# ChainSafe/co-zkvms

Hardware: AMD Instinct MI355X
Metric: RISC-V cycles proved/sec (co-Jolt hot path: PST13 commit + dense GKR grand product + openings) (higher is better)
Workload: dtype u32-limb BN254 Fr/Fq (254-bit Montgomery integers); 1 GPU; configs[1] restated (SURVEY 8d): 2^20-cycle trace per GPU, plain prover, 128 polys (64 Fr + 32 u16 + 16 u32 + 16 flags) PST13 batch commit, dense grand product 8 x 2^21 leaves, batch evaluate + opening reduction + PST13 open; log_n=20, polys=128, gp_batch=8, parallelism=single GPU, ranks_per_gpu=1

## Files before the change

### co-zkvms_amd/csrc/common.hpp

```cpp
#pragma once
#ifdef COZK_COUNT_COPIES
#include <hip/hip_runtime.h>
#include <map>
#include <string>
#include <cstdio>
#include <mutex>
struct CozkCopyCounter {
    std::map<std::string, unsigned long> m;
    std::mutex mu;
    ~CozkCopyCounter() {
        for (auto& kv : m) fprintf(stderr, "[copies] %8lu  %s\n", kv.second, kv.first.c_str());
    }
};
inline CozkCopyCounter& cozk_copy_counter() { static CozkCopyCounter c; return c; }
inline void cozk_count_copy(const char* what, const char* f, int l) {
    auto& c = cozk_copy_counter();
    std::lock_guard<std::mutex> g(c.mu);
    const char* b = f;
    for (const char* p = f; *p; p++) if (*p == '/') b = p + 1;
    c.m[std::string(what) + " " + b + ":" + std::to_string(l)]++;
}
#define hipMemcpyAsync(...) (cozk_count_copy("memcpy", __FILE__, __LINE__), hipMemcpyAsync(__VA_ARGS__))
#define hipStreamSynchronize(...) (cozk_count_copy("sync", __FILE__, __LINE__), hipStreamSynchronize(__VA_ARGS__))
#define hipMemsetAsync(...) (cozk_count_copy("memset", __FILE__, __LINE__), hipMemsetAsync(__VA_ARGS__))
// ... 186 lines not shown
    ProfSlot prof_slots[COZK_PROF_SLOTS];
    void* ring_comm = nullptr;
    int ring_rank = 0, ring_n = 0;
    uint64_t ring_bytes = 0;
};

struct ProfScope {
    cozk_ctx* ctx;
    hipStream_t st;
    int slot;
    hipEvent_t e0 = nullptr, e1 = nullptr;
    ProfScope(cozk_ctx* c, int slot_, uint64_t alg_bytes, hipStream_t stream = nullptr) : ctx(c), st(stream ? stream : c->stream), slot(slot_) {
        if (!ctx->prof_enabled) return;
        if (hipEventCreate(&e0) != hipSuccess || hipEventCreate(&e1) != hipSuccess) {
            e0 = e1 = nullptr;
            return;
        }
        (void)hipEventRecord(e0, st);
        ctx->prof_slots[slot].launches += 1;
        ctx->prof_slots[slot].alg_bytes += alg_bytes;
    }
    ~ProfScope() {
        if (!e0) return;
        (void)hipEventRecord(e1, st);
        ctx->prof_slots[slot].events.push_back({e0, e1});
    }
};

struct cozk_bases {
    cozk_ctx* ctx;
    size_t n;
    int nwin;
    g1_affine* table;
    bool has_inf = true;
};

struct cozk_vec {
    cozk_ctx* ctx;
    size_t n;
    int kind;
    void* d;
    size_t bytes;
    bool owned;
};

static inline size_t scalar_kind_bytes(int kind) {
    switch (kind) {
        case COZK_SCALAR_FR: return 32;
        case COZK_SCALAR_U8: return 1;
        case COZK_SCALAR_U16: return 2;
        case COZK_SCALAR_U32: return 4;
        case COZK_SCALAR_U64: return 8;
        case COZK_SCALAR_I64: return 8;
        default: return 0;
    }
}

inline std::mutex g_ctx_mu;
inline std::unordered_set<cozk_ctx*> g_live_ctx;
inline thread_local cozk_ctx* t_cur_ctx = nullptr;
static inline void trim_current_pool() {
    if (t_cur_ctx) t_cur_ctx->pool.trim();
}
static inline bool ctx_is_live(cozk_ctx* ctx) {
    std::lock_guard<std::mutex> lk(g_ctx_mu);
    return g_live_ctx.count(ctx) != 0;
// ... 56 lines not shown
```

### co-zkvms_amd/csrc/msm.hip

```cpp
#include "common.hpp"
#include "fq9.hip.hpp"

static constexpr uint32_t NB = 1u << 15;
static constexpr int CH = 16;
static constexpr int TPB = 256;

template <int KIND>
struct ScalarKind;
template <>
struct ScalarKind<COZK_SCALAR_FR> {
    static constexpr int NWIN = 16;
    static __device__ __forceinline__ bool load(const void* p, size_t i, uint32_t w[8]) {
        fe s = Fr::from_mont(fe_load(reinterpret_cast<const fe*>(p) + i));
#pragma unroll
        for (int k = 0; k < 8; k++) w[k] = s.l[k];
        return false;
    }
};
template <>
struct ScalarKind<COZK_SCALAR_U8> {
    static constexpr int NWIN = 1;
    static __device__ __forceinline__ bool load(const void* p, size_t i, uint32_t w[8]) {
        w[0] = reinterpret_cast<const uint8_t*>(p)[i];
        return false;
// ... 21 lines not shown
    static constexpr int NWIN = 5;
    static __device__ __forceinline__ bool load(const void* p, size_t i, uint32_t w[8]) {
        uint64_t v = reinterpret_cast<const uint64_t*>(p)[i];
        w[0] = (uint32_t)v;
        w[1] = (uint32_t)(v >> 32);
        w[2] = 0;
        return false;
    }
};
template <>
struct ScalarKind<COZK_SCALAR_I64> {
    static constexpr int NWIN = 5;
    static __device__ __forceinline__ bool load(const void* p, size_t i, uint32_t w[8]) {
        int64_t v = reinterpret_cast<const int64_t*>(p)[i];
        bool neg = v < 0;
        uint64_t m = neg ? (uint64_t)0 - (uint64_t)v : (uint64_t)v;
        w[0] = (uint32_t)m;
        w[1] = (uint32_t)(m >> 32);
        w[2] = 0;
        return neg;
    }
};

static inline int kind_nwin(int kind) {
    switch (kind) {
        case COZK_SCALAR_FR: return 16;
        case COZK_SCALAR_U8: return 1;
        case COZK_SCALAR_U16: return 2;
        case COZK_SCALAR_U32: return 3;
        default: return 5;
    }
}

template <int KIND, class F>
__device__ __forceinline__ void for_each_digit(const void* scalars, size_t i, F&& f) {
    uint32_t w[8] = {0, 0, 0, 0, 0, 0, 0, 0};
    bool neg = ScalarKind<KIND>::load(scalars, i, w);
    uint32_t carry = 0;
#pragma unroll
    for (int k = 0; k < ScalarKind<KIND>::NWIN; k++) {
        uint32_t v = ((w[k >> 1] >> (16 * (k & 1))) & 0xffffu) + carry;
        bool sub = v > 32768u;
        carry = sub ? 1u : 0u;
        uint32_t mag = sub ? 65536u - v : v;
        f(k, mag, sub != neg);
    }
}

static __device__ __forceinline__ uint32_t agg_atomic_add(uint32_t* counters, uint32_t key, bool active) {
    uint64_t act = __ballot(active);
    uint32_t pos = 0;
    if (act == 0) return 0;
    int lane = threadIdx.x & 63;
    int first = __ffsll((unsigned long long)act) - 1;
    uint32_t k0 = __shfl(key, first);
    uint64_t same = __ballot(active && key == k0);
    int cnt = __popcll(same);
    bool merged = false;
    if (cnt >= 4) {
        uint32_t base = 0;
        if (lane == first) base = atomicAdd(&counters[k0], (uint32_t)cnt);
        base = __shfl(base, first);
        if (active && key == k0) {
            pos = base + __popcll(same & ((1ull << lane) - 1ull));
            merged = true;
        }
    }
    if (active && !merged) pos = atomicAdd(&counters[key], 1u);
    return pos;
}
// ... 2 lines not shown
__global__ void __launch_bounds__(TPB) k_msm_hist(const void* scalars, size_t n, uint32_t* hist, int grouped) {
    size_t i = (size_t)blockIdx.x * TPB + threadIdx.x;
    bool inr = i < n;
    size_t ii = inr ? i : 0;
    for_each_digit<KIND>(scalars, ii, [&](int k, uint32_t mag, bool) {
        bool act = inr && mag != 0;
        uint32_t key = (grouped ? (uint32_t)k * NB : 0u) + (mag - 1u);
        agg_atomic_add(hist, act ? key : 0u, act);
    });
}

template <int KIND>
__global__ void __launch_bounds__(TPB) k_msm_scatter(const void* scalars, size_t n, uint32_t* cursor, uint32_t* refs,
                                                  int grouped, uint32_t table_n, uint32_t base_off) {
    size_t i = (size_t)blockIdx.x * TPB + threadIdx.x;
    bool inr = i < n;
    size_t ii = inr ? i : 0;
    for_each_digit<KIND>(scalars, ii, [&](int k, uint32_t mag, bool negative) {
        bool act = inr && mag != 0;
        uint32_t key = (grouped ? (uint32_t)k * NB : 0u) + (mag - 1u);
        uint32_t pos = agg_atomic_add(cursor, act ? key : 0u, act);
        if (act) {
            uint32_t ref = (grouped ? 0u : (uint32_t)k * table_n) + base_off + (uint32_t)ii;
            refs[pos] = ref | (negative ? 0x80000000u : 0u);
        }
    });
}

struct MsmPolyDesc {
    const void* scalars;
    uint32_t n;
    uint32_t base_off;
    uint32_t group;
    uint32_t pad;
};
static constexpr int LTPB = 1024;

template <int KIND>
__global__ void __launch_bounds__(LTPB) k_msm_hist_lds(const MsmPolyDesc* __restrict__ descs, uint32_t* __restrict__ hist) {
    __shared__ uint32_t lh[NB];
    const MsmPolyDesc d = descs[blockIdx.y];
    for (uint32_t b = threadIdx.x; b < NB; b += blockDim.x) lh[b] = 0;
    __syncthreads();
    for (size_t i = (size_t)blockIdx.x * blockDim.x + threadIdx.x; i < d.n; i += (size_t)gridDim.x * blockDim.x) {
        for_each_digit<KIND>(d.scalars, i, [&](int, uint32_t mag, bool) {
            if (mag != 0) atomicAdd(&lh[mag - 1u], 1u);
        });
    }
    __syncthreads();
    uint32_t* h = hist + (size_t)d.group * NB;
    for (uint32_t b = threadIdx.x; b < NB; b += blockDim.x) {
        uint32_t c = lh[b];
        if (c) atomicAdd(&h[b], c);
    }
}

template <int KIND>
__global__ void __launch_bounds__(LTPB) k_msm_scatter_lds(const MsmPolyDesc* __restrict__ descs, uint32_t* __restrict__ cursor,
                                                       uint32_t* __restrict__ refs, uint32_t table_n) {
    __shared__ uint32_t lh[NB];
    const MsmPolyDesc d = descs[blockIdx.y];
    for (uint32_t b = threadIdx.x; b < NB; b += blockDim.x) lh[b] = 0;
    __syncthreads();
    for (size_t i = (size_t)blockIdx.x * blockDim.x + threadIdx.x; i < d.n; i += (size_t)gridDim.x * blockDim.x) {
        for_each_digit<KIND>(d.scalars, i, [&](int, uint32_t mag, bool) {
            if (mag != 0) atomicAdd(&lh[mag - 1u], 1u);
        });
    }
    __syncthreads();
    uint32_t* cur = cursor + (size_t)d.group * NB;
    for (uint32_t b = threadIdx.x; b < NB; b += blockDim.x) {
        uint32_t c = lh[b];
        lh[b] = c ? atomicAdd(&cur[b], c) : 0u;
    }
    __syncthreads();
    for (size_t i = (size_t)blockIdx.x * blockDim.x + threadIdx.x; i < d.n; i += (size_t)gridDim.x * blockDim.x) {
        for_each_digit<KIND>(d.scalars, i, [&](int k, uint32_t mag, bool negative) {
            if (mag != 0) {
                uint32_t pos = atomicAdd(&lh[mag - 1u], 1u);
                uint32_t ref = (uint32_t)k * table_n + d.base_off + (uint32_t)i;
                refs[pos] = ref | (negative ? 0x80000000u : 0u);
            }
        });
    }
}

static constexpr uint32_t SCAN_PER_BLOCK = 1024;

template <bool FROM_OFFSETS>
static __device__ __forceinline__ void scan_load4(const uint32_t* __restrict__ in, uint32_t nb, uint32_t L, uint32_t b0, uint32_t c[4],
                                                  const uint32_t* __restrict__ perm) {
#pragma unroll
    for (int k = 0; k < 4; k++) {
        uint32_t b = b0 + k;
        if (b >= nb) c[k] = 0;
        else if (FROM_OFFSETS) {
            uint32_t q = perm ? perm[b] : b;
            c[k] = (in[q + 1] - in[q] + L - 1u) / L;
        } else c[k] = in[b];
    }
}

static __device__ __forceinline__ uint32_t block_exclusive_scan_256(uint32_t v, uint32_t* sh4, uint32_t* total) {
    uint32_t x = v;
#pragma unroll
    for (int off = 1; off < 64; off <<= 1) {
        uint32_t y = __shfl_up(x, off);
        if ((int)(threadIdx.x & 63) >= off) x += y;
    }
    int w = threadIdx.x >> 6;
    if ((threadIdx.x & 63) == 63) sh4[w] = x;
    __syncthreads();
    uint32_t base = 0;
    for (int i = 0; i < w; i++) base += sh4[i];
    if (total) *total = sh4[0] + sh4[1] + sh4[2] + sh4[3];
    __syncthreads();
    return base + x - v;
// ... 317 lines not shown
    g1_xyzz acc = G1::identity();
    for (uint32_t c = tid; c < cpg; c += TPB) acc = G1::add(acc, xyzz_load(chunk + (size_t)g * cpg + c));
    sh[tid] = acc;
    __syncthreads();
    for (uint32_t s = TPB / 2; s > 0; s >>= 1) {
        if (tid < s) {
            acc = G1::add(acc, sh[tid + s]);
            sh[tid] = acc;
        }
        __syncthreads();
    }
    if (tid == 0) xyzz_store(grp + g, acc);
}

__global__ void k_msm_finalize(const g1_xyzz* __restrict__ grp, uint32_t G, uint32_t npoly, g1_affine* __restrict__ out) {
    uint32_t p = blockIdx.x * blockDim.x + threadIdx.x;
    if (p >= npoly) return;
    g1_xyzz acc = xyzz_load(grp + (size_t)p * G + (G - 1));
    for (int w = (int)G - 2; w >= 0; w--) {
        for (int d = 0; d < 16; d++) acc = G1::dbl(acc);
        acc = G1::add(acc, xyzz_load(grp + (size_t)p * G + w));
    }
    affine_store(out + p, G1::to_affine(acc));
}

__global__ void __launch_bounds__(TPB) k_precompute_window(const g1_affine* __restrict__ prev, g1_affine* __restrict__ next, size_t n) {
    size_t i = (size_t)blockIdx.x * TPB + threadIdx.x;
    if (i >= n) return;
    g1_xyzz acc = G1::dbl_affine(affine_load(prev + i));
    for (int d = 1; d < 16; d++) acc = G1::dbl(acc);
    affine_store(next + i, G1::to_affine(acc));
}

__global__ void __launch_bounds__(TPB) k_fixed_base_mul(const fe* __restrict__ scalars, g1_affine g, g1_affine* __restrict__ out, size_t n) {
    size_t i = (size_t)blockIdx.x * TPB + threadIdx.x;
    if (i >= n) return;
    fe s = Fr::from_mont(fe_load(scalars + i));
    g1_xyzz acc = G1::identity();
    for (int k = 7; k >= 0; k--) {
        uint32_t w = s.l[k];
        for (int b = 31; b >= 0; b--) {
            acc = G1::dbl(acc);
            if ((w >> b) & 1u) acc = G1::add_mixed(acc, g);
        }
    }
    affine_store(out + i, G1::to_affine(acc));
}

__global__ void __launch_bounds__(TPB) k_pair_sums(const g1_affine* __restrict__ in, g1_affine* __restrict__ out, size_t nout) {
    size_t i = (size_t)blockIdx.x * TPB + threadIdx.x;
    if (i >= nout) return;
    g1_xyzz acc = G1::from_affine(affine_load(in + 2 * i));
    acc = G1::add_mixed(acc, affine_load(in + 2 * i + 1));
    affine_store(out + i, G1::to_affine(acc));
}

static inline uint32_t cdiv(uint64_t a, uint64_t b) { return (uint32_t)((a + b - 1) / b); }

__global__ void __launch_bounds__(TPB) k_any_infinity(const g1_affine* __restrict__ pts, size_t n, uint32_t* __restrict__ flag) {
    size_t i = (size_t)blockIdx.x * TPB + threadIdx.x;
    if (i < n && G1::is_inf(affine_load(pts + i))) atomicOr(flag, 1u);
}
static void build_window_table(cozk_ctx* ctx, cozk_bases* b) {
    for (int w = 1; w < b->nwin; w++) {
        k_precompute_window<<<cdiv(b->n, TPB), TPB, 0, ctx->stream>>>(b->table + (size_t)(w - 1) * b->n,
                                                                     b->table + (size_t)w * b->n, b->n);
    }
    HIP_TRY(hipGetLastError());
    ctx->scratch.reserve(64);
    uint32_t* flag = ctx->scratch.as<uint32_t>();
    HIP_TRY(hipMemsetAsync(flag, 0, 4, ctx->stream));
    k_any_infinity<<<cdiv(b->n, TPB), TPB, 0, ctx->stream>>>(b->table, b->n, flag);
    uint32_t h = 1;
    HIP_TRY(hipMemcpyAsync(&h, flag, 4, hipMemcpyDeviceToHost, ctx->stream));
    HIP_TRY(hipStreamSynchronize(ctx->stream));
    b->has_inf = h != 0;
}

#define KIND_DISPATCH(kind, CALL)                                              \
    switch (kind) {                                                            \
        case COZK_SCALAR_FR: { constexpr int K = COZK_SCALAR_FR; CALL; } break;   \
        case COZK_SCALAR_U8: { constexpr int K = COZK_SCALAR_U8; CALL; } break;   \
        case COZK_SCALAR_U16: { constexpr int K = COZK_SCALAR_U16; CALL; } break; \
        case COZK_SCALAR_U32: { constexpr int K = COZK_SCALAR_U32; CALL; } break; \
        case COZK_SCALAR_U64: { constexpr int K = COZK_SCALAR_U64; CALL; } break; \
        case COZK_SCALAR_I64: { constexpr int K = COZK_SCALAR_I64; CALL; } break; \
        default: throw CozkError(COZK_ERR_INVALID_ARG, "unknown scalar kind");    \
    }

struct MsmSetPlan {
    uint32_t P = 0, G = 1, nb = 0, L0 = 8;
    uint64_t M = 0, bound = 0, maxseg0 = 0;
    bool pre = false;
};

static MsmSetPlan msm_plan(const cozk_bases* bases, const size_t* offsets, const size_t* ns, const int* kinds, size_t P) {
    COZK_REQUIRE(P >= 1, "msm: empty batch");
    COZK_REQUIRE((uint64_t)bases->n * (uint64_t)bases->nwin < (1ull << 31), "msm: table too large for 31-bit refs");
    MsmSetPlan pl;
    pl.P = (uint32_t)P;
    pl.pre = bases->nwin == 16;
    pl.G = pl.pre ? 1u : 16u;
    pl.nb = (uint32_t)P * pl.G * NB;
    for (size_t p = 0; p < P; p++) {
        COZK_REQUIRE(offsets[p] + ns[p] <= bases->n, "msm: base slice out of range");
        uint64_t m = (uint64_t)ns[p] * kind_nwin(kinds[p]);
        pl.M += m;
        if (m > pl.bound) pl.bound = m;
    }
    COZK_REQUIRE(pl.M < (1ull << 32), "msm: batch too large (reference count exceeds 32 bits)");
    uint32_t L0 = (uint32_t)(pl.M >> 18);
    if (L0 < 8) L0 = 8;
    if (L0 > 127) L0 = 127;
    pl.L0 = L0;
    pl.maxseg0 = pl.M / L0 + pl.nb;
    return pl;
}

static void msm_scan(hipStream_t st, uint32_t* bsums, uint32_t nb, bool from_offsets, const uint32_t* in, uint32_t L, uint32_t* off, uint32_t* cursor,
                     const uint32_t* perm = nullptr) {
    const uint32_t nscan_blocks = (nb + SCAN_PER_BLOCK - 1) / SCAN_PER_BLOCK;
    if (from_offsets) {
        k_scan_sums<true><<<nscan_blocks, 256, 0, st>>>(in, nb, L, bsums, perm);
        k_scan_top<<<1, 1024, 0, st>>>(bsums, nscan_blocks, off + nb);
        k_scan_final<true><<<nscan_blocks, 256, 0, st>>>(in, nb, L, bsums, off, cursor, perm);
    } else {
        k_scan_sums<false><<<nscan_blocks, 256, 0, st>>>(in, nb, L, bsums, nullptr);
        k_scan_top<<<1, 1024, 0, st>>>(bsums, nscan_blocks, off + nb);
        k_scan_final<false><<<nscan_blocks, 256, 0, st>>>(in, nb, L, bsums, off, cursor, nullptr);
    }
}

static void msm_sort(cozk_ctx* ctx, hipStream_t st, MsmSortWs& sw, const MsmSetPlan& pl, const cozk_bases* bases, const size_t* offsets,
                     const size_t* ns, const void* const* scalars, const int* kinds) {
    const uint32_t nb = pl.nb, G = pl.G;
    const size_t P = pl.P;
    sw.hist.reserve((size_t)(nb + 2) * 4);
    sw.off0.reserve((size_t)(nb + 1) * 4);
    sw.offA.reserve((size_t)(nb + 1) * 4);
    sw.refs.reserve((size_t)pl.M * 4);
    uint32_t* hist = sw.hist.as<uint32_t>();
    uint32_t* off0 = sw.off0.as<uint32_t>();
    uint32_t* refs = sw.refs.as<uint32_t>();
    const uint32_t nscan_blocks = (nb + SCAN_PER_BLOCK - 1) / SCAN_PER_BLOCK;
    sw.ptrs.reserve((size_t)nscan_blocks * 4 + P * sizeof(MsmPolyDesc) + 64);
    uint32_t* bsums = sw.ptrs.as<uint32_t>();
    MsmPolyDesc* d_descs = reinterpret_cast<MsmPolyDesc*>(((uintptr_t)(bsums + nscan_blocks) + 15) & ~(uintptr_t)15);
    HIP_TRY(hipMemsetAsync(hist, 0, (size_t)(nb + 2) * 4, st));
    uint32_t* d_maxcnt = hist + nb + 1;
    if (!sw.max_pinned) HIP_TRY(hipHostMalloc((void**)&sw.max_pinned, 64 + 64 * sizeof(MsmPolyDesc), hipHostMallocDefault));
    if (!sw.max_event) HIP_TRY(hipEventCreateWithFlags(&sw.max_event, hipEventDisableTiming));
    auto read_back_max = [&] {
        k_max_u32<<<std::min<uint32_t>(cdiv(nb, 256), 1024u), 256, 0, st>>>(hist, nb, d_maxcnt);
        HIP_TRY(hipMemcpyAsync(sw.max_pinned, d_maxcnt, 4, hipMemcpyDeviceToHost, st));
        HIP_TRY(hipEventRecord(sw.max_event, st));
    };
    if (pl.pre) {
        MsmPolyDesc* h_descs = reinterpret_cast<MsmPolyDesc*>(reinterpret_cast<char*>(sw.max_pinned) + 64);
        COZK_REQUIRE(P <= 64, "msm: too many polynomials in one launch set");
        uint32_t nd = 0;
        std::vector<std::pair<int, std::pair<uint32_t, uint32_t>>> runs;
        size_t max_n = 0;
        for (int kind = 0; kind <= COZK_SCALAR_I64; kind++) {
            uint32_t first = nd;
            for (size_t p = 0; p < P; p++)
                if (kinds[p] == kind && ns[p]) {
                    h_descs[nd++] = MsmPolyDesc{scalars[p], (uint32_t)ns[p], (uint32_t)offsets[p], (uint32_t)p, 0};
                    if (ns[p] > max_n) max_n = ns[p];
                }
            if (nd > first) runs.push_back({kind, {first, nd - first}});
        }
        HIP_TRY(hipMemcpyAsync(d_descs, h_descs, nd * sizeof(MsmPolyDesc), hipMemcpyHostToDevice, st));
        static const int ltpb = getenv("COZK_MSM_LTPB") ? atoi(getenv("COZK_MSM_LTPB")) : 256;
        static const uint32_t wgs_max = getenv("COZK_MSM_WGS") ? (uint32_t)atoi(getenv("COZK_MSM_WGS")) : 64u;
        COZK_REQUIRE(ltpb >= 64 && ltpb <= LTPB && ltpb % 64 == 0, "COZK_MSM_LTPB out of range");
        COZK_REQUIRE(wgs_max >= 1 && wgs_max <= 1024, "COZK_MSM_WGS out of range (1..1024)");
        uint32_t wgs = (uint32_t)((max_n + 4095) / 4096);
        if (wgs < 1) wgs = 1;
        if (wgs > wgs_max) wgs = wgs_max;
        for (auto& r : runs) {
            dim3 grid(wgs, r.second.second);
            KIND_DISPATCH(r.first, (k_msm_hist_lds<K><<<grid, ltpb, 0, st>>>(d_descs + r.second.first, hist)));
        }
        read_back_max();
        msm_scan(st, bsums, nb, false, hist, 1, off0, hist);
        for (auto& r : runs) {
            dim3 grid(wgs, r.second.second);
            uint64_t alg = 0;
            for (uint32_t q = 0; q < r.second.second; q++) {
                const MsmPolyDesc& d = h_descs[r.second.first + q];
                const uint64_t sb = scalar_kind_bytes(r.first);
                alg += (uint64_t)d.n * (sb + 4ull * ((sb * 8 + 15) / 16));
            }
            ProfScope prof(ctx, COZK_PROF_MSM_SCATTER, alg, st);
            KIND_DISPATCH(r.first, (k_msm_scatter_lds<K><<<grid, ltpb, 0, st>>>(d_descs + r.second.first, hist, refs, (uint32_t)bases->n)));
        }
    } else {
        for (size_t p = 0; p < P; p++) {
            uint32_t* h = hist + (size_t)p * G * NB;
            if (ns[p]) KIND_DISPATCH(kinds[p], (k_msm_hist<K><<<cdiv(ns[p], TPB), TPB, 0, st>>>(scalars[p], ns[p], h, 1)));
        }
        read_back_max();
        msm_scan(st, bsums, nb, false, hist, 1, off0, hist);
        for (size_t p = 0; p < P; p++) {
            uint32_t* cur = hist + (size_t)p * G * NB;
            if (ns[p])
                KIND_DISPATCH(kinds[p], (k_msm_scatter<K><<<cdiv(ns[p], TPB), TPB, 0, st>>>(scalars[p], ns[p], cur, refs, 1, (uint32_t)bases->n,
                                                                                         (uint32_t)offsets[p])));
        }
    }
    msm_scan(st, bsums, nb, true, off0, pl.L0, sw.offA.as<uint32_t>(), nullptr);
    HIP_TRY(hipGetLastError());
}

static void msm_accumulate(cozk_ctx* ctx, MsmSortWs& sw, const MsmSetPlan& pl, const cozk_bases* bases, const size_t* ns, const int* kinds,
                           g1_xyzz* dense_out) {
    MsmWorkspace& ws = ctx->msm_ws;
    hipStream_t st = ctx->stream;
    const uint32_t nb = pl.nb, L0 = pl.L0;
    const uint32_t L1 = 8;
    const uint64_t maxseg0 = pl.maxseg0;
    const uint64_t maxpart = maxseg0 > 2ull * nb ? maxseg0 : 2ull * nb;
    ws.partA.reserve((size_t)maxpart * sizeof(g1_xyzz));
    ws.partB.reserve((size_t)maxpart * sizeof(g1_xyzz));
    ws.offB.reserve((size_t)(nb + 1) * 4);
    ws.offC.reserve((size_t)(nb + 1) * 4);
    ws.ptrs.reserve((size_t)((nb + SCAN_PER_BLOCK - 1) / SCAN_PER_BLOCK) * 4 + 64);
    uint32_t* refs = sw.refs.as<uint32_t>();
    uint32_t* off0 = sw.off0.as<uint32_t>();
    uint32_t* offA = sw.offA.as<uint32_t>();
    hipEvent_t e0 = nullptr, e1 = nullptr;
    if (ctx->prof_enabled) {
        HIP_TRY(hipEventCreate(&e0));
        HIP_TRY(hipEventCreate(&e1));
        HIP_TRY(hipEventRecord(e0, st));
    }
    ws.blk.reserve((size_t)(cdiv(maxpart, TPB) + 2) * 4);
    uint32_t* blk = ws.blk.as<uint32_t>();
    if (pl.pre) {
        ws.exc.reserve((size_t)(maxseg0 + 2) * 4);
        uint32_t* exc = ws.exc.as<uint32_t>();
        HIP_TRY(hipMemsetAsync(exc, 0, 4, st));
        ws.perm.reserve((size_t)nb * 4);
        ws.offP.reserve((size_t)(nb + 1) * 4 + SEGKEYS * 4);
        uint32_t* perm = ws.perm.as<uint32_t>();
        uint32_t* offP = ws.offP.as<uint32_t>();
        uint32_t* bins = offP + nb + 1;
        HIP_TRY(hipMemsetAsync(bins, 0, SEGKEYS * 4, st));
        k_seg_hist<<<cdiv(nb, 1024), 1024, 0, st>>>(off0, offA, nb, bins);
        k_seg_bins<<<1, 1, 0, st>>>(bins);
        k_seg_perm<<<cdiv(nb, 1024), 1024, 0, st>>>(off0, offA, nb, bins, perm);
        msm_scan(st, ws.ptrs.as<uint32_t>(), nb, true, offA, 1, offP, nullptr, perm);
        const uint32_t nblk0 = cdiv(maxseg0, TPB);
        k_block_buckets<<<cdiv(nblk0 + 1, 256), 256, 0, st>>>(offP, nb, nblk0, blk);
        if (bases->has_inf)
            k_msm_accum0_f9<true><<<nblk0, TPB, 0, st>>>(bases->table, refs, off0, offA, nb, ws.partA.as<g1_xyzz>(), exc, blk, offP, perm);
        else
            k_msm_accum0_f9<false, true><<<nblk0, TPB, 0, st>>>(bases->table, refs, off0, offA, nb, ws.partA.as<g1_xyzz>(), exc, blk, offP, perm);
        k_msm_accum0_fix<<<256, TPB, 0, st>>>(bases->table, refs, off0, offA, nb, ws.partA.as<g1_xyzz>(), exc, offP, perm);
    } else {
        k_msm_accum0<<<cdiv(maxseg0, TPB), TPB, 0, st>>>(bases->table, refs, off0, offA, nb, L0, ws.partA.as<g1_xyzz>());
    }
    if (ctx->prof_enabled) {
        HIP_TRY(hipEventRecord(e1, st));
        ctx->prof_events.push_back({e0, e1});
        ctx->prof_launches += 1;
        ctx->prof_units += pl.M;
        for (size_t p = 0; p < pl.P; p++) ctx->prof_alg_bytes += (uint64_t)ns[p] * (64 + scalar_kind_bytes(kinds[p]));
    }
    HIP_TRY(hipEventSynchronize(sw.max_event));
    uint64_t fullest = *(volatile uint32_t*)sw.max_pinned;
    COZK_REQUIRE(fullest <= pl.bound, "msm: histogram larger than the reference count");
    uint64_t cnt = (fullest + L0 - 1) / L0;
    uint64_t maxseg = maxseg0;
    g1_xyzz* cur_items = ws.partA.as<g1_xyzz>();
    g1_xyzz* nxt_items = ws.partB.as<g1_xyzz>();
    uint32_t* cur_off = offA;
    uint32_t* nxt_off = ws.offB.as<uint32_t>();
    uint32_t* spare_off = ws.offC.as<uint32_t>();
    while (cnt > 1) {
        uint64_t nseg = maxseg / L1 + nb;
        msm_scan(st, ws.ptrs.as<uint32_t>(), nb, true, cur_off, L1, nxt_off, nullptr);
        const uint32_t nblkN = cdiv(nseg, TPB);
        k_block_buckets<<<cdiv(nblkN + 1, 256), 256, 0, st>>>(nxt_off, nb, nblkN, blk);
        k_msm_accumN<<<nblkN, TPB, 0, st>>>(cur_items, cur_off, nxt_off, nb, L1, nxt_items, blk);
        std::swap(cur_items, nxt_items);
        uint32_t* done = cur_off;
        cur_off = nxt_off;
        nxt_off = (done == offA) ? spare_off : done;
        maxseg = nseg;
        cnt = (cnt + L1 - 1) / L1;
    }
    k_msm_gather_buckets<<<cdiv(nb, TPB), TPB, 0, st>>>(cur_items, cur_off, nb, dense_out);
    HIP_TRY(hipGetLastError());
// ... 30 lines not shown
    const size_t maxP = bases->nwin == 16 ? 64 : 4;
    const size_t tail_cap = 256 / G;
    ws.out.reserve(k * sizeof(g1_affine));
    g1_affine* d_out = ws.out.as<g1_affine>();
    for (size_t t0 = 0; t0 < k; t0 += tail_cap) {
        size_t kt = k - t0 < tail_cap ? k - t0 : tail_cap;
        const uint32_t ngroups = (uint32_t)kt * G;
        ws.bsum.reserve((size_t)ngroups * NB * sizeof(g1_xyzz));
        ws.chunk.reserve((size_t)ngroups * (NB / CH) * sizeof(g1_xyzz));
        ws.grp.reserve((size_t)ngroups * sizeof(g1_xyzz));
        g1_xyzz* dense = ws.bsum.as<g1_xyzz>();
        struct SetRange { size_t s, P; };
        std::vector<SetRange> sets;
        uint64_t set_refs_cap;
        {
            static const int pinned = getenv("COZK_MSM_SET_REFS_LOG2") ? atoi(getenv("COZK_MSM_SET_REFS_LOG2")) : 0;
            if (pinned) set_refs_cap = 1ull << (pinned < 24 ? 24 : (pinned > 31 ? 31 : pinned));
            else {
                uint64_t total = 0;
                for (size_t p = 0; p < kt; p++) total += (uint64_t)ns[t0 + p] * kind_nwin(kinds[t0 + p]);
                set_refs_cap = total / 4;
                if (set_refs_cap < (1ull << 28)) set_refs_cap = 1ull << 28;
                if (set_refs_cap > (1ull << 30)) set_refs_cap = 1ull << 30;
            }
        }
        {
            size_t s = 0;
            while (s < kt) {
                size_t P = 0;
                uint64_t M = 0;
                while (s + P < kt && P < maxP) {
                    uint64_t m = (uint64_t)ns[t0 + s + P] * kind_nwin(kinds[t0 + s + P]);
                    if (P > 0 && M + m > set_refs_cap) break;
                    M += m;
                    P++;
                }
                sets.push_back({s, P});
                s += P;
            }
        }
        if (sets.size() > 2) {
            size_t best = 0;
            uint64_t best_m = ~0ull;
            for (size_t i = 0; i < sets.size(); i++) {
                uint64_t m = 0;
                for (size_t p = 0; p < sets[i].P; p++) m += (uint64_t)ns[t0 + sets[i].s + p] * kind_nwin(kinds[t0 + sets[i].s + p]);
                if (m < best_m) {
                    best_m = m;
                    best = i;
                }
            }
            std::rotate(sets.begin(), sets.begin() + best, sets.begin() + best + 1);
        }
        static const bool pipeline = getenv("COZK_MSM_SERIAL") == nullptr;
        hipStream_t side = st;
        if (pipeline && sets.size() > 1) {
            if (!ctx->stream2) {
                static const bool prio = getenv("COZK_MSM_NO_PRIORITY") == nullptr;
                int lo = 0, hi = 0;
                HIP_TRY(hipDeviceGetStreamPriorityRange(&lo, &hi));
                if (prio) HIP_TRY(hipStreamCreateWithPriority(&ctx->stream2, hipStreamNonBlocking, hi));
                else HIP_TRY(hipStreamCreateWithFlags(&ctx->stream2, hipStreamNonBlocking));
            }
            side = ctx->stream2;
        }
        for (int b = 0; b < 2; b++) {
// ... 17 lines not shown
        };
        if (!sets.empty()) launch_sort(0);
        for (size_t i = 0; i < sets.size(); i++) {
            if (side != st && i + 1 < sets.size()) launch_sort(i + 1);
            const SetRange& r = sets[i];
            g1_xyzz* out_i = dense + (size_t)r.s * G * NB;
            if (plans[i].M != 0) {
                MsmSortWs& sw = ws.sort[i & 1];
                if (side != st) HIP_TRY(hipStreamWaitEvent(st, sw.done, 0));
                msm_accumulate(ctx, sw, plans[i], bases, ns + t0 + r.s, kinds + t0 + r.s, out_i);
                if (side != st) HIP_TRY(hipEventRecord(sw.consumed, st));
            } else {
                HIP_TRY(hipMemsetAsync(out_i, 0, (size_t)plans[i].nb * sizeof(g1_xyzz), st));
            }
            if (side == st && i + 1 < sets.size()) launch_sort(i + 1);
        }
        k_msm_reduce_chunks<<<cdiv((uint64_t)ngroups * (NB / CH), TPB), TPB, 0, st>>>(dense, ngroups, ws.chunk.as<g1_xyzz>());
        k_msm_reduce_groups<<<ngroups, TPB, 0, st>>>(ws.chunk.as<g1_xyzz>(), ws.grp.as<g1_xyzz>());
        k_msm_finalize<<<cdiv(kt, 64), 64, 0, st>>>(ws.grp.as<g1_xyzz>(), G, (uint32_t)kt, d_out + t0);
        HIP_TRY(hipGetLastError());
    }
    g1_affine* h = reinterpret_cast<g1_affine*>(ctx_pinned(ctx, k * sizeof(g1_affine)));
    HIP_TRY(hipMemcpyAsync(h, d_out, k * sizeof(g1_affine), hipMemcpyDeviceToHost, st));
    HIP_TRY(hipStreamSynchronize(st));
    for (size_t i = 0; i < k; i++) affine_to_abi(h[i], out_xy + 8 * i, out_inf ? out_inf + i : nullptr);
}

extern "C" {

int cozk_bases_upload(cozk_ctx* ctx, const uint64_t* xy, const uint8_t* infinity, size_t n, int precompute,
                      cozk_bases** out) {
    return cozk_guard(ctx, [&] {
        COZK_REQUIRE(ctx && xy && out && n > 0, "bases_upload: bad argument");
        cozk_bases* b = new cozk_bases{ctx, n, precompute ? 16 : 1, nullptr};
        try {
            HIP_TRY(hipMalloc((void**)&b->table, (size_t)b->nwin * n * sizeof(g1_affine)));
            std::vector<g1_affine> h(n);
            for (size_t i = 0; i < n; i++) h[i] = abi_to_affine(xy + 8 * i, infinity ? infinity[i] : 0);
            HIP_TRY(hipMemcpyAsync(b->table, h.data(), n * sizeof(g1_affine), hipMemcpyHostToDevice, ctx->stream));
            HIP_TRY(hipStreamSynchronize(ctx->stream));
            build_window_table(ctx, b);
            HIP_TRY(hipStreamSynchronize(ctx->stream));
        } catch (...) {
            if (b->table) (void)hipFree(b->table);
            delete b;
            throw;
        }
        *out = b;
    });
}

int cozk_bases_from_scalars(cozk_ctx* ctx, const cozk_vec* s, const uint64_t* g_xy, int precompute, cozk_bases** out) {
    return cozk_guard(ctx, [&] {
        COZK_REQUIRE(ctx && s && g_xy && out && s->kind == COZK_SCALAR_FR && s->n > 0, "bases_from_scalars: bad argument");
        size_t n = s->n;
        cozk_bases* b = new cozk_bases{ctx, n, precompute ? 16 : 1, nullptr};
        try {
            HIP_TRY(hipMalloc((void**)&b->table, (size_t)b->nwin * n * sizeof(g1_affine)));
            g1_affine g = abi_to_affine(g_xy, 0);
            k_fixed_base_mul<<<cdiv(n, TPB), TPB, 0, ctx->stream>>>(reinterpret_cast<const fe*>(s->d), g, b->table, n);
            HIP_TRY(hipGetLastError());
            build_window_table(ctx, b);
            HIP_TRY(hipStreamSynchronize(ctx->stream));
        } catch (...) {
            if (b->table) (void)hipFree(b->table);
            delete b;
            throw;
        }
        *out = b;
    });
}

int cozk_bases_pair_sums(cozk_ctx* ctx, const cozk_bases* src, int precompute, cozk_bases** out) {
    return cozk_guard(ctx, [&] {
        COZK_REQUIRE(ctx && src && out && src->n >= 2 && src->n % 2 == 0, "bases_pair_sums: bad argument");
        size_t n = src->n / 2;
        cozk_bases* b = new cozk_bases{ctx, n, precompute ? 16 : 1, nullptr};
        try {
            HIP_TRY(hipMalloc((void**)&b->table, (size_t)b->nwin * n * sizeof(g1_affine)));
            k_pair_sums<<<cdiv(n, TPB), TPB, 0, ctx->stream>>>(src->table, b->table, n);
            HIP_TRY(hipGetLastError());
            build_window_table(ctx, b);
            HIP_TRY(hipStreamSynchronize(ctx->stream));
        } catch (...) {
            if (b->table) (void)hipFree(b->table);
            delete b;
            throw;
        }
        *out = b;
    });
}

int cozk_bases_download(cozk_ctx* ctx, const cozk_bases* b, size_t offset, size_t n, uint64_t* xy, uint8_t* infinity) {
    return cozk_guard(ctx, [&] {
        COZK_REQUIRE(ctx && b && xy && offset + n <= b->n, "bases_download: bad argument");
        std::vector<g1_affine> h(n);
        HIP_TRY(hipMemcpyAsync(h.data(), b->table + offset, n * sizeof(g1_affine), hipMemcpyDeviceToHost, ctx->stream));
        HIP_TRY(hipStreamSynchronize(ctx->stream));
        for (size_t i = 0; i < n; i++) {
            int inf;
            affine_to_abi(h[i], xy + 8 * i, &inf);
            if (infinity) infinity[i] = (uint8_t)inf;
        }
    });
}

int cozk_bases_free(cozk_bases* b) {
    if (!b) return COZK_OK;
    if (b->table) (void)hipFree(b->table);
    delete b;
    return COZK_OK;
}
// ... 150 lines not shown
```

### co-zkvms_amd/engine.py

```python
import ctypes

import numpy as np

from . import _lib as L

FR_MOD = 21888242871839275222246405745257275088548364400416034343698204186575808495617
FQ_MOD = 21888242871839275222246405745257275088696311157297823662689037894645226208583
_MONT = 1 << 256
_MASK64 = (1 << 64) - 1

_KIND_DTYPE = {L.SCALAR_U8: np.uint8, L.SCALAR_U16: np.uint16, L.SCALAR_U32: np.uint32,
               L.SCALAR_U64: np.uint64, L.SCALAR_I64: np.int64}


def fr_to_mont_limbs(values, mod=FR_MOD):
    out = np.empty((len(values), 4), dtype=np.uint64)
    for i, v in enumerate(values):
        m = (int(v) % mod) * _MONT % mod
        out[i, 0] = m & _MASK64
        out[i, 1] = (m >> 64) & _MASK64
        out[i, 2] = (m >> 128) & _MASK64
        out[i, 3] = (m >> 192) & _MASK64
    return out

# ... 529 lines not shown
    party_ctxs[0].check(party_ctxs[0]._l.cozk_shamir_gp_prep_inproc(ctxs, rk, n_leaves, batch_size, degree, n, rand_counter, ctypes.byref(h)))
    return ShamirGpPrep(party_ctxs, h, degree)


def shamir_gp_prove_king(party_ctxs, leaves, batch_size, prep, king=0, label=b"cozk", verify=True):
    n = len(party_ctxs)
    l = party_ctxs[0]._l
    ctxs = (ctypes.c_void_p * max(n, 1))(*[c.h for c in party_ctxs])
    h = ctypes.c_void_p()
    party_ctxs[0].check(l.cozk_shamir_gp_prove_king_inproc(ctxs, _handles(n, leaves), batch_size, prep.h, king, bytes(label), 1 if verify else 0,
                                                           ctypes.byref(h)))
    try:
        return ShamirGpProof(l, h, prep.degree)
    finally:
        l.cozk_shamir_gp_free(h)


def shamir_combine_points(ctx, points_g1, points, degree):
    k = len(points_g1)
    xy = np.zeros((max(k, 1), 8), dtype=np.uint64)
    inf = np.zeros(max(k, 1), dtype=np.int32)
    for i, p in enumerate(points_g1):
        xy[i], inf[i] = point_to_abi(p)
    pts = _points(points)
    out = np.zeros(8, dtype=np.uint64)
    oi = ctypes.c_int()
    ctx.check(ctx._l.cozk_shamir_combine_points(ctx.h, xy.ctypes.data, inf.ctypes.data, pts.ctypes.data, k, degree, out.ctypes.data,
                                                ctypes.byref(oi)))
    return point_from_abi(out, oi.value)


class Bases:

    def __init__(self, ctx, handle):
        self.ctx = ctx
        self.h = handle

    @classmethod
    def upload(cls, ctx, points, precompute=True):
        n = len(points)
        xy = np.zeros((n, 8), dtype=np.uint64)
        inf = np.zeros(n, dtype=np.uint8)
        for i, p in enumerate(points):
            xy[i], inf[i] = point_to_abi(p)
        h = ctypes.c_void_p()
        ctx.check(ctx._l.cozk_bases_upload(ctx.h, xy.ctypes.data, inf.ctypes.data, n, 1 if precompute else 0,
                                           ctypes.byref(h)))
        return cls(ctx, h)

    @classmethod
    def from_scalars(cls, ctx, scalars_vec, g=(1, 2), precompute=True):
        gxy, _ = point_to_abi(g)
        h = ctypes.c_void_p()
        ctx.check(ctx._l.cozk_bases_from_scalars(ctx.h, scalars_vec.h, gxy.ctypes.data, 1 if precompute else 0,
                                                 ctypes.byref(h)))
        return cls(ctx, h)

    def pair_sums(self, precompute=True):
        h = ctypes.c_void_p()
        self.ctx.check(self.ctx._l.cozk_bases_pair_sums(self.ctx.h, self.h, 1 if precompute else 0, ctypes.byref(h)))
        return Bases(self.ctx, h)

    def __len__(self):
        return self.ctx._l.cozk_bases_len(self.h)

    def download(self, offset=0, n=None):
        if n is None:
            n = len(self) - offset
        xy = np.zeros((n, 8), dtype=np.uint64)
        inf = np.zeros(n, dtype=np.uint8)
        self.ctx.check(self.ctx._l.cozk_bases_download(self.ctx.h, self.h, offset, n, xy.ctypes.data, inf.ctypes.data))
        return [point_from_abi(xy[i], inf[i]) for i in range(n)]

    def msm(self, scalars, offset=0):
        out = np.zeros(8, dtype=np.uint64)
        oi = ctypes.c_int()
        self.ctx.check(self.ctx._l.cozk_msm_vec(self.ctx.h, self.h, offset, scalars.h, out.ctypes.data, ctypes.byref(oi)))
        return point_from_abi(out, oi.value)

    def msm_host(self, arr, kind=L.SCALAR_FR, offset=0):
        arr = np.ascontiguousarray(arr)
        n = arr.shape[0]
        out = np.zeros(8, dtype=np.uint64)
        oi = ctypes.c_int()
        self.ctx.check(self.ctx._l.cozk_msm(self.ctx.h, self.h, offset, arr.ctypes.data if n else None, kind, n,
                                            out.ctypes.data, ctypes.byref(oi)))
        return point_from_abi(out, oi.value)

    def batch_msm_raw(self, vecs, offset=0):
        k = len(vecs)
        arr = (ctypes.c_void_p * k)(*[v.h for v in vecs])
        out = np.zeros((k, 8), dtype=np.uint64)
        inf = np.zeros(k, dtype=np.int32)
        self.ctx.check(self.ctx._l.cozk_batch_msm_vec(self.ctx.h, self.h, offset, arr, k, out.ctypes.data,
# ... 18 lines not shown
```

Baseline: 9.087 million cycles/s.

## Use raw Montgomery limbs as MSM digits via R^-1-scaled base table

Adds a second precomputed window table whose bases are scaled by R^-1, so field scalars in Montgomery form can be decomposed into digits directly without a from_mont conversion in every histogram and scatter pass. Also sizes per-polynomial workgroup counts from digit count instead of one global max, shrinks the LDS histogram for u8 scalars, and uses wave-aggregated LDS atomics for narrow scalar kinds. The cost is twice the device memory for precomputed bases plus extra setup kernels, and launch sets can no longer mix field and narrow scalars.

```diff
diff --git a/co-zkvms_amd/csrc/common.hpp b/co-zkvms_amd/csrc/common.hpp
--- a/co-zkvms_amd/csrc/common.hpp
+++ b/co-zkvms_amd/csrc/common.hpp
@@ -242,6 +242,8 @@
     size_t n;
     int nwin;
     g1_affine* table;
+    g1_affine* table_raw = nullptr;
+    size_t device_bytes = 0;
     bool has_inf = true;
 };
 
diff --git a/co-zkvms_amd/csrc/msm.hip b/co-zkvms_amd/csrc/msm.hip
--- a/co-zkvms_amd/csrc/msm.hip
+++ b/co-zkvms_amd/csrc/msm.hip
@@ -77,10 +77,30 @@
     }
 }
 
-template <int KIND, class F>
+struct FrRawLimbs {
+    static constexpr int NWIN = 16;
+    static __device__ __forceinline__ bool load(const void* p, size_t i, uint32_t w[8]) {
+        fe s = fe_load(reinterpret_cast<const fe*>(p) + i);
+#pragma unroll
+        for (int k = 0; k < 8; k++) w[k] = s.l[k];
+        return false;
+    }
+};
+template <int KIND, bool RAW>
+struct DigitSource {
+    using type = ScalarKind<KIND>;
+};
+template <>
+struct DigitSource<COZK_SCALAR_FR, true> {
+    using type = FrRawLimbs;
+};
+
+template <int KIND, bool RAW = false, class F>
 __device__ __forceinline__ void for_each_digit(const void* scalars, size_t i, F&& f) {
+    static_assert(!RAW || KIND == COZK_SCALAR_FR, "raw-limb digits exist for field scalars only");
+    using Src = typename DigitSource<KIND, RAW>::type;
     uint32_t w[8] = {0, 0, 0, 0, 0, 0, 0, 0};
-    bool neg = ScalarKind<KIND>::load(scalars, i, w);
+    bool neg = Src::load(scalars, i, w);
     uint32_t carry = 0;
 #pragma unroll
     for (int k = 0; k < ScalarKind<KIND>::NWIN; k++) {
@@ -149,57 +169,81 @@
     uint32_t n;
     uint32_t base_off;
     uint32_t group;
-    uint32_t pad;
+    uint32_t wgs;
 };
 static constexpr int LTPB = 1024;
 
 template <int KIND>
+static constexpr uint32_t KIND_NB = KIND == COZK_SCALAR_U8 ? 255u : NB;
+template <int KIND>
+static constexpr bool KIND_HOT = KIND != COZK_SCALAR_FR;
+
+template <int KIND, bool RAW, bool PLACE>
+static __device__ __forceinline__ void lds_digit_pass(const MsmPolyDesc& d, uint32_t* lh, uint32_t* __restrict__ refs, uint32_t table_n) {
+    const size_t stride = (size_t)d.wgs * blockDim.x;
+    if constexpr (KIND_HOT<KIND>) {
+        for (size_t i0 = (size_t)blockIdx.x * blockDim.x + (threadIdx.x & ~63u); i0 < d.n; i0 += stride) {
+            const size_t i = i0 + (threadIdx.x & 63u);
+            const bool inr = i < d.n;
+            for_each_digit<KIND, RAW>(d.scalars, inr ? i : 0, [&](int k, uint32_t mag, bool negative) {
+                const bool act = inr && mag != 0;
+                uint32_t pos = agg_atomic_add(lh, act ? mag - 1u : 0u, act);
+                if (PLACE && act) {
+                    uint32_t ref = (uint32_t)k * table_n + d.base_off + (uint32_t)i;
+                    refs[pos] = ref | (negative ? 0x80000000u : 0u);
+                }
+            });
+        }
+    } else {
+        for (size_t i = (size_t)blockIdx.x * blockDim.x + threadIdx.x; i < d.n; i += stride) {
+            for_each_digit<KIND, RAW>(d.scalars, i, [&](int k, uint32_t mag, bool negative) {
+                if (mag != 0) {
+                    uint32_t pos = atomicAdd(&lh[mag - 1u], 1u);
+                    if (PLACE) {
+                        uint32_t ref = (uint32_t)k * table_n + d.base_off + (uint32_t)i;
+                        refs[pos] = ref | (negative ? 0x80000000u : 0u);
+                    }
+                }
+            });
+        }
+    }
+}
+
+template <int KIND, bool RAW = false>
 __global__ void __launch_bounds__(LTPB) k_msm_hist_lds(const MsmPolyDesc* __restrict__ descs, uint32_t* __restrict__ hist) {
     __shared__ uint32_t lh[NB];
     const MsmPolyDesc d = descs[blockIdx.y];
-    for (uint32_t b = threadIdx.x; b < NB; b += blockDim.x) lh[b] = 0;
-    __syncthreads();
-    for (size_t i = (size_t)blockIdx.x * blockDim.x + threadIdx.x; i < d.n; i += (size_t)gridDim.x * blockDim.x) {
-        for_each_digit<KIND>(d.scalars, i, [&](int, uint32_t mag, bool) {
-            if (mag != 0) atomicAdd(&lh[mag - 1u], 1u);
-        });
-    }
+    if (blockIdx.x >= d.wgs) return;
+    constexpr uint32_t nbk = KIND_NB<KIND>;
+    for (uint32_t b = threadIdx.x; b < nbk; b += blockDim.x) lh[b] = 0;
+    __syncthreads();
+    lds_digit_pass<KIND, RAW, false>(d, lh, nullptr, 0);
     __syncthreads();
     uint32_t* h = hist + (size_t)d.group * NB;
-    for (uint32_t b = threadIdx.x; b < NB; b += blockDim.x) {
+    for (uint32_t b = threadIdx.x; b < nbk; b += blockDim.x) {
         uint32_t c = lh[b];
         if (c) atomicAdd(&h[b], c);
     }
 }
 
-template <int KIND>
+template <int KIND, bool RAW = false>
 __global__ void __launch_bounds__(LTPB) k_msm_scatter_lds(const MsmPolyDesc* __restrict__ descs, uint32_t* __restrict__ cursor,
                                                        uint32_t* __restrict__ refs, uint32_t table_n) {
     __shared__ uint32_t lh[NB];
     const MsmPolyDesc d = descs[blockIdx.y];
-    for (uint32_t b = threadIdx.x; b < NB; b += blockDim.x) lh[b] = 0;
-    __syncthreads();
-    for (size_t i = (size_t)blockIdx.x * blockDim.x + threadIdx.x; i < d.n; i += (size_t)gridDim.x * blockDim.x) {
-        for_each_digit<KIND>(d.scalars, i, [&](int, uint32_t mag, bool) {
-            if (mag != 0) atomicAdd(&lh[mag - 1u], 1u);
-        });
-    }
+    if (blockIdx.x >= d.wgs) return;
+    constexpr uint32_t nbk = KIND_NB<KIND>;
+    for (uint32_t b = threadIdx.x; b < nbk; b += blockDim.x) lh[b] = 0;
+    __syncthreads();
+    lds_digit_pass<KIND, RAW, false>(d, lh, nullptr, 0);
     __syncthreads();
     uint32_t* cur = cursor + (size_t)d.group * NB;
-    for (uint32_t b = threadIdx.x; b < NB; b += blockDim.x) {
+    for (uint32_t b = threadIdx.x; b < nbk; b += blockDim.x) {
         uint32_t c = lh[b];
         lh[b] = c ? atomicAdd(&cur[b], c) : 0u;
     }
     __syncthreads();
-    for (size_t i = (size_t)blockIdx.x * blockDim.x + threadIdx.x; i < d.n; i += (size_t)gridDim.x * blockDim.x) {
-        for_each_digit<KIND>(d.scalars, i, [&](int k, uint32_t mag, bool negative) {
-            if (mag != 0) {
-                uint32_t pos = atomicAdd(&lh[mag - 1u], 1u);
-                uint32_t ref = (uint32_t)k * table_n + d.base_off + (uint32_t)i;
-                refs[pos] = ref | (negative ? 0x80000000u : 0u);
-            }
-        });
-    }
+    lds_digit_pass<KIND, RAW, true>(d, lh, refs, table_n);
 }
 
 static constexpr uint32_t SCAN_PER_BLOCK = 1024;
@@ -583,10 +627,12 @@
     affine_store(next + i, G1::to_affine(acc));
 }
 
+template <bool RINV>
 __global__ void __launch_bounds__(TPB) k_fixed_base_mul(const fe* __restrict__ scalars, g1_affine g, g1_affine* __restrict__ out, size_t n) {
     size_t i = (size_t)blockIdx.x * TPB + threadIdx.x;
     if (i >= n) return;
     fe s = Fr::from_mont(fe_load(scalars + i));
+    if (RINV) s = Fr::from_mont(s);
     g1_xyzz acc = G1::identity();
     for (int k = 7; k >= 0; k--) {
         uint32_t w = s.l[k];
@@ -598,6 +644,28 @@
     affine_store(out + i, G1::to_affine(acc));
 }
 
+__global__ void __launch_bounds__(TPB) k_scale_rinv(const g1_affine* __restrict__ table, g1_affine* __restrict__ out, size_t n) {
+    size_t i = (size_t)blockIdx.x * TPB + threadIdx.x;
+    if (i >= n) return;
+    g1_affine p0 = affine_load(table + i);
+    if (G1::is_inf(p0)) {
+        affine_store(out + i, p0);
+        return;
+    }
+    fe c;
+    c.l[0] = 1;
+#pragma unroll
+    for (int k = 1; k < 8; k++) c.l[k] = 0;
+    c = Fr::from_mont(c);
+    g1_xyzz acc = G1::identity();
+    for (int b = 15; b >= 0; b--) {
+        acc = G1::dbl(acc);
+        for (int w = 0; w < 16; w++)
+            if ((c.l[w >> 1] >> (16 * (w & 1) + b)) & 1u) acc = G1::add_mixed(acc, affine_load(table + (size_t)w * n + i));
+    }
+    affine_store(out + i, G1::to_affine(acc));
+}
+
 __global__ void __launch_bounds__(TPB) k_pair_sums(const g1_affine* __restrict__ in, g1_affine* __restrict__ out, size_t nout) {
     size_t i = (size_t)blockIdx.x * TPB + threadIdx.x;
     if (i >= nout) return;
@@ -612,10 +680,27 @@
     size_t i = (size_t)blockIdx.x * TPB + threadIdx.x;
     if (i < n && G1::is_inf(affine_load(pts + i))) atomicOr(flag, 1u);
 }
-static void build_window_table(cozk_ctx* ctx, cozk_bases* b) {
-    for (int w = 1; w < b->nwin; w++) {
-        k_precompute_window<<<cdiv(b->n, TPB), TPB, 0, ctx->stream>>>(b->table + (size_t)(w - 1) * b->n,
-                                                                     b->table + (size_t)w * b->n, b->n);
+static cozk_bases* bases_alloc(cozk_ctx* ctx, size_t n, int precompute) {
+    cozk_bases* b = new cozk_bases{ctx, n, precompute ? 16 : 1, nullptr};
+    b->device_bytes = (size_t)(precompute ? 32 : 1) * n * sizeof(g1_affine);
+    try {
+        HIP_TRY(hipMalloc((void**)&b->table, b->device_bytes));
+    } catch (...) {
+        delete b;
+        throw;
+    }
+    if (precompute) b->table_raw = b->table + (size_t)16 * n;
+    return b;
+}
+static void build_window_table(cozk_ctx* ctx, cozk_bases* b, const fe* from_scalars = nullptr, const g1_affine* g = nullptr) {
+    const uint32_t nblk = cdiv(b->n, TPB);
+    for (int w = 1; w < b->nwin; w++)
+        k_precompute_window<<<nblk, TPB, 0, ctx->stream>>>(b->table + (size_t)(w - 1) * b->n, b->table + (size_t)w * b->n, b->n);
+    if (b->table_raw) {
+        if (from_scalars) k_fixed_base_mul<true><<<nblk, TPB, 0, ctx->stream>>>(from_scalars, *g, b->table_raw, b->n);
+        else k_scale_rinv<<<nblk, TPB, 0, ctx->stream>>>(b->table, b->table_raw, b->n);
+        for (int w = 1; w < 16; w++)
+            k_precompute_window<<<nblk, TPB, 0, ctx->stream>>>(b->table_raw + (size_t)(w - 1) * b->n, b->table_raw + (size_t)w * b->n, b->n);
     }
     HIP_TRY(hipGetLastError());
     ctx->scratch.reserve(64);
@@ -643,6 +728,7 @@
     uint32_t P = 0, G = 1, nb = 0, L0 = 8;
     uint64_t M = 0, bound = 0, maxseg0 = 0;
     bool pre = false;
+    bool raw = false;
 };
 
 static MsmSetPlan msm_plan(const cozk_bases* bases, const size_t* offsets, const size_t* ns, const int* kinds, size_t P) {
@@ -651,10 +737,12 @@
     MsmSetPlan pl;
     pl.P = (uint32_t)P;
     pl.pre = bases->nwin == 16;
+    pl.raw = pl.pre && kinds[0] == COZK_SCALAR_FR;
     pl.G = pl.pre ? 1u : 16u;
     pl.nb = (uint32_t)P * pl.G * NB;
     for (size_t p = 0; p < P; p++) {
         COZK_REQUIRE(offsets[p] + ns[p] <= bases->n, "msm: base slice out of range");
+        COZK_REQUIRE(!pl.pre || (kinds[p] == COZK_SCALAR_FR) == pl.raw, "msm: launch set mixes field and narrow scalars");
         uint64_t m = (uint64_t)ns[p] * kind_nwin(kinds[p]);
         pl.M += m;
         if (m > pl.bound) pl.bound = m;
@@ -711,32 +799,39 @@
         COZK_REQUIRE(P <= 64, "msm: too many polynomials in one launch set");
         uint32_t nd = 0;
         std::vector<std::pair<int, std::pair<uint32_t, uint32_t>>> runs;
-        size_t max_n = 0;
+        static const int ltpb = getenv("COZK_MSM_LTPB") ? atoi(getenv("COZK_MSM_LTPB")) : 256;
+        static const uint32_t wgs_max = getenv("COZK_MSM_WGS") ? (uint32_t)atoi(getenv("COZK_MSM_WGS")) : 64u;
+        static const int wg_digits_log2 = getenv("COZK_MSM_WG_DIGITS_LOG2") ? atoi(getenv("COZK_MSM_WG_DIGITS_LOG2")) : 16;
+        COZK_REQUIRE(ltpb >= 64 && ltpb <= LTPB && ltpb % 64 == 0, "COZK_MSM_LTPB out of range");
+        COZK_REQUIRE(wgs_max >= 1 && wgs_max <= 1024, "COZK_MSM_WGS out of range (1..1024)");
+        COZK_REQUIRE(wg_digits_log2 >= 12 && wg_digits_log2 <= 20, "COZK_MSM_WG_DIGITS_LOG2 out of range (12..20)");
+        std::vector<uint32_t> run_wgs;
         for (int kind = 0; kind <= COZK_SCALAR_I64; kind++) {
-            uint32_t first = nd;
+            uint32_t first = nd, widest = 1;
             for (size_t p = 0; p < P; p++)
                 if (kinds[p] == kind && ns[p]) {
-                    h_descs[nd++] = MsmPolyDesc{scalars[p], (uint32_t)ns[p], (uint32_t)offsets[p], (uint32_t)p, 0};
-                    if (ns[p] > max_n) max_n = ns[p];
+                    uint64_t w = ((uint64_t)ns[p] * kind_nwin(kind) + (1ull << wg_digits_log2) - 1) >> wg_digits_log2;
+                    uint32_t wgs = (uint32_t)std::min<uint64_t>(std::max<uint64_t>(w, 1), wgs_max);
+                    h_descs[nd++] = MsmPolyDesc{scalars[p], (uint32_t)ns[p], (uint32_t)offsets[p], (uint32_t)p, wgs};
+                    widest = std::max(widest, wgs);
                 }
-            if (nd > first) runs.push_back({kind, {first, nd - first}});
+            if (nd > first) {
+                runs.push_back({kind, {first, nd - first}});
+                run_wgs.push_back(widest);
+            }
         }
         HIP_TRY(hipMemcpyAsync(d_descs, h_descs, nd * sizeof(MsmPolyDesc), hipMemcpyHostToDevice, st));
-        static const int ltpb = getenv("COZK_MSM_LTPB") ? atoi(getenv("COZK_MSM_LTPB")) : 256;
-        static const uint32_t wgs_max = getenv("COZK_MSM_WGS") ? (uint32_t)atoi(getenv("COZK_MSM_WGS")) : 64u;
-        COZK_REQUIRE(ltpb >= 64 && ltpb <= LTPB && ltpb % 64 == 0, "COZK_MSM_LTPB out of range");
-        COZK_REQUIRE(wgs_max >= 1 && wgs_max <= 1024, "COZK_MSM_WGS out of range (1..1024)");
-        uint32_t wgs = (uint32_t)((max_n + 4095) / 4096);
-        if (wgs < 1) wgs = 1;
-        if (wgs > wgs_max) wgs = wgs_max;
-        for (auto& r : runs) {
-            dim3 grid(wgs, r.second.second);
-            KIND_DISPATCH(r.first, (k_msm_hist_lds<K><<<grid, ltpb, 0, st>>>(d_descs + r.second.first, hist)));
+        for (size_t ri = 0; ri < runs.size(); ri++) {
+            auto& r = runs[ri];
+            dim3 grid(run_wgs[ri], r.second.second);
+            if (pl.raw) k_msm_hist_lds<COZK_SCALAR_FR, true><<<grid, ltpb, 0, st>>>(d_descs + r.second.first, hist);
+            else KIND_DISPATCH(r.first, (k_msm_hist_lds<K><<<grid, ltpb, 0, st>>>(d_descs + r.second.first, hist)));
         }
         read_back_max();
         msm_scan(st, bsums, nb, false, hist, 1, off0, hist);
-        for (auto& r : runs) {
-            dim3 grid(wgs, r.second.second);
+        for (size_t ri = 0; ri < runs.size(); ri++) {
+            auto& r = runs[ri];
+            dim3 grid(run_wgs[ri], r.second.second);
             uint64_t alg = 0;
             for (uint32_t q = 0; q < r.second.second; q++) {
                 const MsmPolyDesc& d = h_descs[r.second.first + q];
@@ -744,7 +839,8 @@
                 alg += (uint64_t)d.n * (sb + 4ull * ((sb * 8 + 15) / 16));
             }
             ProfScope prof(ctx, COZK_PROF_MSM_SCATTER, alg, st);
-            KIND_DISPATCH(r.first, (k_msm_scatter_lds<K><<<grid, ltpb, 0, st>>>(d_descs + r.second.first, hist, refs, (uint32_t)bases->n)));
+            if (pl.raw) k_msm_scatter_lds<COZK_SCALAR_FR, true><<<grid, ltpb, 0, st>>>(d_descs + r.second.first, hist, refs, (uint32_t)bases->n);
+            else KIND_DISPATCH(r.first, (k_msm_scatter_lds<K><<<grid, ltpb, 0, st>>>(d_descs + r.second.first, hist, refs, (uint32_t)bases->n)));
         }
     } else {
         for (size_t p = 0; p < P; p++) {
@@ -780,6 +876,7 @@
     uint32_t* refs = sw.refs.as<uint32_t>();
     uint32_t* off0 = sw.off0.as<uint32_t>();
     uint32_t* offA = sw.offA.as<uint32_t>();
+    const g1_affine* table = pl.raw ? bases->table_raw : bases->table;
     hipEvent_t e0 = nullptr, e1 = nullptr;
     if (ctx->prof_enabled) {
         HIP_TRY(hipEventCreate(&e0));
@@ -805,12 +902,12 @@
         const uint32_t nblk0 = cdiv(maxseg0, TPB);
         k_block_buckets<<<cdiv(nblk0 + 1, 256), 256, 0, st>>>(offP, nb, nblk0, blk);
         if (bases->has_inf)
-            k_msm_accum0_f9<true><<<nblk0, TPB, 0, st>>>(bases->table, refs, off0, offA, nb, ws.partA.as<g1_xyzz>(), exc, blk, offP, perm);
+            k_msm_accum0_f9<true><<<nblk0, TPB, 0, st>>>(table, refs, off0, offA, nb, ws.partA.as<g1_xyzz>(), exc, blk, offP, perm);
         else
-            k_msm_accum0_f9<false, true><<<nblk0, TPB, 0, st>>>(bases->table, refs, off0, offA, nb, ws.partA.as<g1_xyzz>(), exc, blk, offP, perm);
-        k_msm_accum0_fix<<<256, TPB, 0, st>>>(bases->table, refs, off0, offA, nb, ws.partA.as<g1_xyzz>(), exc, offP, perm);
+            k_msm_accum0_f9<false, true><<<nblk0, TPB, 0, st>>>(table, refs, off0, offA, nb, ws.partA.as<g1_xyzz>(), exc, blk, offP, perm);
+        k_msm_accum0_fix<<<256, TPB, 0, st>>>(table, refs, off0, offA, nb, ws.partA.as<g1_xyzz>(), exc, offP, perm);
     } else {
-        k_msm_accum0<<<cdiv(maxseg0, TPB), TPB, 0, st>>>(bases->table, refs, off0, offA, nb, L0, ws.partA.as<g1_xyzz>());
+        k_msm_accum0<<<cdiv(maxseg0, TPB), TPB, 0, st>>>(table, refs, off0, offA, nb, L0, ws.partA.as<g1_xyzz>());
     }
     if (ctx->prof_enabled) {
         HIP_TRY(hipEventRecord(e1, st));
@@ -907,6 +1004,7 @@
                 while (s + P < kt && P < maxP) {
                     uint64_t m = (uint64_t)ns[t0 + s + P] * kind_nwin(kinds[t0 + s + P]);
                     if (P > 0 && M + m > set_refs_cap) break;
+                    if (P > 0 && G == 1 && (kinds[t0 + s + P] == COZK_SCALAR_FR) != (kinds[t0 + s] == COZK_SCALAR_FR)) break;
                     M += m;
                     P++;
                 }
@@ -990,9 +1088,8 @@
                       cozk_bases** out) {
     return cozk_guard(ctx, [&] {
         COZK_REQUIRE(ctx && xy && out && n > 0, "bases_upload: bad argument");
-        cozk_bases* b = new cozk_bases{ctx, n, precompute ? 16 : 1, nullptr};
+        cozk_bases* b = bases_alloc(ctx, n, precompute);
         try {
-            HIP_TRY(hipMalloc((void**)&b->table, (size_t)b->nwin * n * sizeof(g1_affine)));
             std::vector<g1_affine> h(n);
             for (size_t i = 0; i < n; i++) h[i] = abi_to_affine(xy + 8 * i, infinity ? infinity[i] : 0);
             HIP_TRY(hipMemcpyAsync(b->table, h.data(), n * sizeof(g1_affine), hipMemcpyHostToDevice, ctx->stream));
@@ -1012,13 +1109,12 @@
     return cozk_guard(ctx, [&] {
         COZK_REQUIRE(ctx && s && g_xy && out && s->kind == COZK_SCALAR_FR && s->n > 0, "bases_from_scalars: bad argument");
         size_t n = s->n;
-        cozk_bases* b = new cozk_bases{ctx, n, precompute ? 16 : 1, nullptr};
+        cozk_bases* b = bases_alloc(ctx, n, precompute);
         try {
-            HIP_TRY(hipMalloc((void**)&b->table, (size_t)b->nwin * n * sizeof(g1_affine)));
             g1_affine g = abi_to_affine(g_xy, 0);
-            k_fixed_base_mul<<<cdiv(n, TPB), TPB, 0, ctx->stream>>>(reinterpret_cast<const fe*>(s->d), g, b->table, n);
+            k_fixed_base_mul<false><<<cdiv(n, TPB), TPB, 0, ctx->stream>>>(reinterpret_cast<const fe*>(s->d), g, b->table, n);
             HIP_TRY(hipGetLastError());
-            build_window_table(ctx, b);
+            build_window_table(ctx, b, reinterpret_cast<const fe*>(s->d), &g);
             HIP_TRY(hipStreamSynchronize(ctx->stream));
         } catch (...) {
             if (b->table) (void)hipFree(b->table);
@@ -1033,9 +1129,8 @@
     return cozk_guard(ctx, [&] {
         COZK_REQUIRE(ctx && src && out && src->n >= 2 && src->n % 2 == 0, "bases_pair_sums: bad argument");
         size_t n = src->n / 2;
-        cozk_bases* b = new cozk_bases{ctx, n, precompute ? 16 : 1, nullptr};
+        cozk_bases* b = bases_alloc(ctx, n, precompute);
         try {
-            HIP_TRY(hipMalloc((void**)&b->table, (size_t)b->nwin * n * sizeof(g1_affine)));
             k_pair_sums<<<cdiv(n, TPB), TPB, 0, ctx->stream>>>(src->table, b->table, n);
             HIP_TRY(hipGetLastError());
             build_window_table(ctx, b);
diff --git a/co-zkvms_amd/engine.py b/co-zkvms_amd/engine.py
--- a/co-zkvms_amd/engine.py
+++ b/co-zkvms_amd/engine.py
@@ -585,9 +585,14 @@
 
 class Bases:
 
-    def __init__(self, ctx, handle):
+    def __init__(self, ctx, handle, precompute=False):
         self.ctx = ctx
         self.h = handle
+        self.precompute = bool(precompute)
+
+    @property
+    def device_bytes(self):
+        return len(self) * 64 * (32 if self.precompute else 1)
 
     @classmethod
     def upload(cls, ctx, points, precompute=True):
@@ -599,7 +604,7 @@
         h = ctypes.c_void_p()
         ctx.check(ctx._l.cozk_bases_upload(ctx.h, xy.ctypes.data, inf.ctypes.data, n, 1 if precompute else 0,
                                            ctypes.byref(h)))
-        return cls(ctx, h)
+        return cls(ctx, h, precompute)
 
     @classmethod
     def from_scalars(cls, ctx, scalars_vec, g=(1, 2), precompute=True):
@@ -607,12 +612,12 @@
         h = ctypes.c_void_p()
         ctx.check(ctx._l.cozk_bases_from_scalars(ctx.h, scalars_vec.h, gxy.ctypes.data, 1 if precompute else 0,
                                                  ctypes.byref(h)))
-        return cls(ctx, h)
+        return cls(ctx, h, precompute)
 
     def pair_sums(self, precompute=True):
         h = ctypes.c_void_p()
         self.ctx.check(self.ctx._l.cozk_bases_pair_sums(self.ctx.h, self.h, 1 if precompute else 0, ctypes.byref(h)))
-        return Bases(self.ctx, h)
+        return Bases(self.ctx, h, precompute)
 
     def __len__(self):
         return self.ctx._l.cozk_bases_len(self.h)
```

Measured after the change: 9.173 million cycles/s (median of 6 runs). Within noise of the previous version (+0.9%).
